# nintendops/DynamicFusion_Body

Hardware: AMD Instinct MI355X
Metric: Mvoxels/s TSDF fusion + GN-iters/s warp solve, 256³ grid, 1/2/4/8 GPU (higher is better)
Workload: dtype f64 geometry / f32 volume

## Files before the change

dynamicfusion_body_amd/csrc/dfh_common.h:

```cpp
#pragma once
#include <hip/hip_runtime.h>

#include <cstdarg>
#include <cstdio>

#include "../../include/dfusion_hip.h"

namespace dfh {

char *last_error_buf();
int fail(int code, const char *fmt, ...);

#define DFH_HIP_CHECK(expr)                                                               \
    do {                                                                                  \
        hipError_t _e = (expr);                                                           \
        if (_e != hipSuccess)                                                             \
            return ::dfh::fail(DFH_E_HIP, "%s failed: %s", #expr, hipGetErrorString(_e)); \
    } while (0)

#define DFH_REQUIRE(cond, ...)                                  \
    do {                                                        \
        if (!(cond)) return ::dfh::fail(DFH_E_BADARG, __VA_ARGS__); \
    } while (0)

inline int check_slab(const char *what, const dfh_slab *s) {
    DFH_REQUIRE(s, "%s: null slab", what);
    DFH_REQUIRE(s->res[0] > 0 && s->res[1] > 0 && s->res[2] > 0, "%s: bad grid %dx%dx%d", what, s->res[0], s->res[1], s->res[2]);
    DFH_REQUIRE(0 <= s->x0 && s->x0 <= s->x1 && s->x1 <= s->res[0], "%s: slab [%d,%d) outside [0,%d)", what, s->x0, s->x1, s->res[0]);
    DFH_REQUIRE(s->x1 - s->x0 <= 65535, "%s: slab has more than 65535 planes", what);
    return DFH_OK;
}

inline int check_volume(const char *what, const dfh_volume *v) {
    DFH_REQUIRE(v && v->tsdf && v->tsdf_w, "%s: null volume", what);
    DFH_REQUIRE(v->dtype == DFH_F32 || v->dtype == DFH_F64, "%s: bad volume dtype %d", what, v->dtype);
    return check_slab(what, &v->slab);
}

struct Mat3 { double m[9]; };
struct Mat34 { double m[12]; };
struct Vec3 { double v[3]; };
struct DQ { double q[8]; };

constexpr int kWave = 64;
#ifndef DFH_GN_TILE
#define DFH_GN_TILE 128
#endif
constexpr int kGnTile = DFH_GN_TILE;

#define DFH_OPTION_LIST(X)                                                                                                \
    X(k1_strided) X(k1_late_loads) X(k1_planes_per_block) X(k1_force_scalar) X(k1_bricks_min) X(k1_no_bricks)            \
    X(k1_bricks_nocull) X(k1_no_multi) X(k1_cull) X(k1_nzi) X(k1_prefetch) X(k1_nt) X(k1_gather_first)                  \
    X(k2_exact) X(k2_no_strided) X(k2_nt) X(k3_no_cache) X(k3_exact) X(k3_no_lds) X(k3_wg_per_cu) X(k3_tpb) X(k3_skip) X(plan_radix) X(rigid_atomic) X(gn_reg_own_launch) X(gn_reg_own_gather) \
    X(dbg_gather_part) X(pcg_wpb) X(pcg_multilaunch) X(pcg_spin_limit) X(pcg_one_xcd) X(gn_iter_own_clear) X(gn_gather_full) X(gn_no_view_cull)                                                            \
    X(py_plan_torch) X(py_allreduce_full) X(py_gn_atomic) X(py_gn_no_fused_assoc) X(py_gn_no_fused_iter) X(py_gn_iter_per_call) X(py_no_side_stream) X(py_no_host_scalars) \
    X(k12_store) X(nd_path) X(raycast_skip)
struct Options {
#define DFH_X(n) long n;
    DFH_OPTION_LIST(DFH_X)
#undef DFH_X
};
const Options &opt();

struct DeviceInfo {
    int n_cu = 0;
    int pcg_occ512 = -1, pcg_occ1024 = -1;
};
DeviceInfo &device_info(int device);
inline bool on(long v) { return v > 0; }

}
```

dynamicfusion_body_amd/csrc/dfh_fuse_volume.hip:

```cpp
#include "dfh_warped_views.h"

#include <algorithm>
#include <cmath>
#include <cstdlib>
#include <mutex>
#include <unordered_map>

namespace dfh {

template <typename T, int N>
struct alignas(sizeof(T) * N) VPack {
    T v[N];
};

struct RigidParams {
    DQ lw;
    double tdist, wmax;
    int X, Y, Z;
    int LX, LY, LZ;
    int x0, nx;
    int zpacks, zp_shift;
};

__device__ __forceinline__ void pack_coords2(int zpacks, int zp_shift, int &y, int &zp) {
    const int lin = blockIdx.x * 256 + threadIdx.x;
    if (zp_shift >= 0) {
        y = lin >> zp_shift;
        zp = lin & ((1 << zp_shift) - 1);
    } else {
        y = lin / zpacks;
        zp = lin - y * zpacks;
    }
}

template <typename VolT, typename LiveT, int VEC>
__global__ __launch_bounds__(256) void fuse_volume_rigid_kernel(VolT *__restrict__ tsdf, VolT *__restrict__ tsdf_w,
                                                                 const LiveT *__restrict__ live, const RigidParams p) {
    int y, zp;
    pack_coords2(p.zpacks, p.zp_shift, y, zp);
    if (y >= p.Y) return;
    const int xl = blockIdx.y;
    const int x = p.x0 + xl;
    const int z0 = zp * VEC;
    double sv[VEC];
    bool upd[VEC];
    bool any = false;
#pragma unroll
    for (int j = 0; j < VEC; ++j) {
        const int z = z0 + j;
        const D3 q = dqb_warp_exact(p.lw.q, (double)x, (double)y, (double)z);
        double s = 0.0;
        bool ok = (z < p.Z) && interpolate_exact(live, p.LX, p.LY, p.LZ, q.x, q.y, q.z, s);
        ok = ok && (s > -1.0 * p.tdist);
        sv[j] = s;
        upd[j] = ok;
        any = any | ok;
    }
    if (!any) return;
    const size_t off = ((size_t)xl * p.Y + y) * p.Z + z0;
    using P = VPack<VolT, VEC>;
    P t = *reinterpret_cast<const P *>(tsdf + off);
    P w = *reinterpret_cast<const P *>(tsdf_w + off);
#pragma unroll
    for (int j = 0; j < VEC; ++j) {
        if (upd[j]) {
            const double wt = (double)w.v[j];
            const double m = sv[j] < p.tdist ? sv[j] : p.tdist;
            t.v[j] = (VolT)(((double)t.v[j] * wt + m * 1.0) / (1.0 + wt));
            const double nw = 1.0 + wt;
            w.v[j] = (VolT)(nw < p.wmax ? nw : p.wmax);
        }
    }
    *reinterpret_cast<P *>(tsdf + off) = t;
    *reinterpret_cast<P *>(tsdf_w + off) = w;
}

struct RigidFastParams {
    double M[9], t[3];
};

template <typename LiveT>
__device__ __forceinline__ double sample_fast(const LiveT *__restrict__ vol, int RY, int RZ, double px, double py, double pz) {
    const double fx = floor(px), fy = floor(py), fz = floor(pz);
    const int x0 = (int)fx, y0 = (int)fy, z0 = (int)fz;
    const int x1 = (int)ceil(px), y1 = (int)ceil(py), z1 = (int)ceil(pz);
    const double xd = px - fx, yd = py - fy, zd = pz - fz;
    const size_t sx = (size_t)RY * RZ, sy = (size_t)RZ;
    const double c000 = (double)vol[x0 * sx + y0 * sy + z0], c100 = (double)vol[x1 * sx + y0 * sy + z0];
    const double c001 = (double)vol[x0 * sx + y1 * sy + z0], c101 = (double)vol[x1 * sx + y1 * sy + z0];
    const double c010 = (double)vol[x0 * sx + y0 * sy + z1], c110 = (double)vol[x1 * sx + y0 * sy + z1];
    const double c011 = (double)vol[x0 * sx + y1 * sy + z1], c111 = (double)vol[x1 * sx + y1 * sy + z1];
    const double c00 = __builtin_fma(xd, c100 - c000, c000), c01 = __builtin_fma(xd, c101 - c001, c001);
    const double c10 = __builtin_fma(xd, c110 - c010, c010), c11 = __builtin_fma(xd, c111 - c011, c011);
    const double c0 = __builtin_fma(yd, c10 - c00, c00);
    const double c1 = __builtin_fma(yd, c11 - c01, c01);
    return __builtin_fma(zd, c1 - c0, c0);
}

template <typename LiveT, bool STRIDED, bool NT = false>
__global__ __launch_bounds__(256) void fuse_volume_rigid_fast_kernel(float *__restrict__ tsdf, float *__restrict__ tsdf_w,
                                                                      const LiveT *__restrict__ live, const RigidParams p,
                                                                      const RigidFastParams f) {
    constexpr int VEC = 4;
    int y, zp;
    pack_coords2(p.zpacks, p.zp_shift, y, zp);
    if (y >= p.Y) return;
    const int xl = blockIdx.y;
    const int x = p.x0 + xl;
    const int lane = threadIdx.x & 63;
    const int z0 = STRIDED ? (zp - lane) * VEC + lane : zp * VEC;
    constexpr int ZS = STRIDED ? 64 : 1;
    const double xf = (double)x, yf = (double)y, zf = (double)z0;
    double q[3];
#pragma unroll
    for (int r = 0; r < 3; ++r)
        q[r] = __builtin_fma(f.M[3 * r + 2], zf, __builtin_fma(f.M[3 * r + 1], yf, __builtin_fma(f.M[3 * r], xf, f.t[r])));
    const double hx = (double)(p.LX - 1), hy = (double)(p.LY - 1), hz = (double)(p.LZ - 1);
    const float tdf = (float)p.tdist;
    float mv[VEC];
    bool upd[VEC];
    bool any = false;
#pragma unroll
    for (int j = 0; j < VEC; ++j) {
        const double jf = (double)(j * ZS);
        const double qx = __builtin_fma(f.M[2], jf, q[0]), qy = __builtin_fma(f.M[5], jf, q[1]), qz = __builtin_fma(f.M[8], jf, q[2]);
        const double lo = fmin(fmin(qx, qy), qz);
        const double hi = fmin(fmin(hx - qx, hy - qy), hz - qz);
        const double edge = fmin(fabs(lo), fabs(hi));
        bool ok = (lo >= 0.0) & (hi >= 0.0);
        bool redo = (int)!(fmin(fmin(fabs(qx), fabs(qy)), fabs(qz)) > 1e-9) | (int)!(fmin(fmin(fabs(hx - qx), fabs(hy - qy)), fabs(hz - qz)) > 1e-9);
        (void)edge;
        double sv = 0.0;
        if (ok) {
            const double fx = qx - floor(qx), fy = qy - floor(qy), fz = qz - floor(qz);
            redo = redo | !(fmin(fmin(fmin(fx, fy), fz), fmin(fmin(1.0 - fx, 1.0 - fy), 1.0 - fz)) > 1e-9);
            sv = sample_fast(live, p.LY, p.LZ, qx, qy, qz);
            const double margin = sv + p.tdist;
            ok = margin > 0.0;
            redo = redo | !(fabs(margin) > 1e-9 * (1.0 + fabs(sv)));
        }
        if (__builtin_expect(redo, 0)) {
            int xx = x, yy = y, zz = z0 + j * ZS;
            asm volatile("" : "+v"(xx), "+v"(yy), "+v"(zz));
            const D3 e = dqb_warp_exact(p.lw.q, (double)xx, (double)yy, (double)zz);
            ok = interpolate_exact(live, p.LX, p.LY, p.LZ, e.x, e.y, e.z, sv) && (sv > -1.0 * p.tdist);
        }
        ok = ok & (z0 + j * ZS < p.Z);
        mv[j] = (float)(sv < p.tdist ? sv : p.tdist);
        upd[j] = ok;
        any = any | ok;
    }
    (void)tdf;
    if (!any) return;
    const size_t off = ((size_t)xl * p.Y + y) * p.Z + z0;
    using P = VPack<float, VEC>;
    P t, w;
    if (STRIDED) {
#pragma unroll
        for (int j = 0; j < VEC; ++j) {
            if (NT) { t.v[j] = __builtin_nontemporal_load(tsdf + off + j * ZS); w.v[j] = __builtin_nontemporal_load(tsdf_w + off + j * ZS); }
            else { t.v[j] = tsdf[off + j * ZS]; w.v[j] = tsdf_w[off + j * ZS]; }
        }
    } else {
        t = *reinterpret_cast<const P *>(tsdf + off);
        w = *reinterpret_cast<const P *>(tsdf_w + off);
    }
    const float wmaxf = (float)p.wmax;
#pragma unroll
    for (int j = 0; j < VEC; ++j) {
        const float wt = w.v[j];
        const float d = wt + 1.0f;
        const float n = fmaf(t.v[j], wt, mv[j]);
        const float r = __builtin_amdgcn_rcpf(d);
        float qn = n * r;
        qn = fmaf(fmaf(-d, qn, n), r, qn);
        t.v[j] = upd[j] ? qn : t.v[j];
        w.v[j] = upd[j] ? fminf(d, wmaxf) : wt;
    }
    if (STRIDED) {
#pragma unroll
        for (int j = 0; j < VEC; ++j) {
            if (upd[j]) {
                if (NT) { __builtin_nontemporal_store(t.v[j], tsdf + off + j * ZS); __builtin_nontemporal_store(w.v[j], tsdf_w + off + j * ZS); }
                else { tsdf[off + j * ZS] = t.v[j]; tsdf_w[off + j * ZS] = w.v[j]; }
            }
        }
    } else {
        *reinterpret_cast<P *>(tsdf + off) = t;
        *reinterpret_cast<P *>(tsdf_w + off) = w;
    }
}

static void fold_rigid(const double *q, RigidFastParams &f) {
    const double w = q[0], x = q[1], y = q[2], z = q[3];
    f.M[0] = w * w + x * x - y * y - z * z; f.M[1] = 2 * (x * y - w * z);           f.M[2] = 2 * (x * z + w * y);
    f.M[3] = 2 * (x * y + w * z);           f.M[4] = w * w - x * x + y * y - z * z; f.M[5] = 2 * (y * z - w * x);
    f.M[6] = 2 * (x * z - w * y);           f.M[7] = 2 * (y * z + w * x);           f.M[8] = w * w - x * x - y * y + z * z;
    const double d0 = q[4], d1 = q[5], d2 = q[6], d3 = q[7];
    f.t[0] = 2 * (-d0 * x + d1 * w - d2 * z + d3 * y);
    f.t[1] = 2 * (-d0 * y + d1 * z + d2 * w - d3 * x);
    f.t[2] = 2 * (-d0 * z - d1 * y + d2 * x + d3 * w);
}

template <typename VolT, typename LiveT>
static int launch_rigid(void *tsdf, void *tsdf_w, const void *live, RigidParams &p, bool vec4, hipStream_t s) {
    p.zpacks = vec4 ? p.Z / 4 : p.Z;
    p.zp_shift = -1;
    for (int b = 0; b < 31; ++b) if (p.zpacks == (1 << b)) p.zp_shift = b;
    const long per_plane = (long)p.Y * p.zpacks;
    dim3 grid((unsigned)((per_plane + 255) / 256), (unsigned)p.nx), block(256);
    if (vec4) {
        hipLaunchKernelGGL((fuse_volume_rigid_kernel<VolT, LiveT, 4>), grid, block, 0, s, (VolT *)tsdf, (VolT *)tsdf_w,
                           (const LiveT *)live, p);
    } else {
        hipLaunchKernelGGL((fuse_volume_rigid_kernel<VolT, LiveT, 1>), grid, block, 0, s, (VolT *)tsdf, (VolT *)tsdf_w,
                           (const LiveT *)live, p);
    }
    DFH_HIP_CHECK(hipGetLastError());
    return DFH_OK;
}

#define DFH_BRICK_RADIUS 7.7942286340599480
#define DFH_SAMPLE_MARGIN 1.7320508075688774

__global__ __launch_bounds__(256) void dqb_candidates_kernel(const double *__restrict__ node_pos, int *__restrict__ cand,
                                                              const DqbParams p) {
    const long brick = (long)blockIdx.x * 256 + threadIdx.x;
    const long nbricks = (long)p.nbx * p.nby * p.nbz;
    if (brick >= nbricks) return;
    const int bz = (int)(brick % p.nbz);
    const int by = (int)((brick / p.nbz) % p.nby);
    const int bx = (int)(brick / ((long)p.nbz * p.nby));
    const double lx = (double)(p.x0 + bx * kBX), ly = (double)(by * kBY), lz = (double)(bz * kBZ);
    const double hx = lx + (kBX - 1), hy = ly + (kBY - 1), hz = lz + (kBZ - 1);
    const double cx = 0.5 * (lx + hx), cy = 0.5 * (ly + hy), cz = 0.5 * (lz + hz);
    double bd[kKMax];
    int bi[kKMax];
#pragma unroll
    for (int i = 0; i < kKMax; ++i) { bd[i] = __builtin_huge_val(); bi[i] = -1; }
    for (int n = 0; n < p.N; ++n) {
        const double dx = cx - node_pos[3 * n], dy = cy - node_pos[3 * n + 1], dz = cz - node_pos[3 * n + 2];
        const double d2 = (dx * dx + dy * dy) + dz * dz;
        if (d2 < bd[kKMax - 1]) topk_insert<kKMax>(bd, bi, d2, n);
    }
    const double R = sqrt(select_k<kKMax>(bd, p.k)) + DFH_BRICK_RADIUS + DFH_SAMPLE_MARGIN + 1e-6;
    const double R2 = R * R;
    int *c = cand + brick * (kCap + 1);
    int cnt = 0;
    for (int n = 0; n < p.N; ++n) {
        const double qx = node_pos[3 * n], qy = node_pos[3 * n + 1], qz = node_pos[3 * n + 2];
        const double dx = fmax(fmax(lx - qx, qx - hx), 0.0), dy = fmax(fmax(ly - qy, qy - hy), 0.0), dz = fmax(fmax(lz - qz, qz - hz), 0.0);
        const double d2 = (dx * dx + dy * dy) + dz * dz;
        if (d2 <= R2) {
            if (cnt < kCap) c[1 + cnt] = n;
            ++cnt;
        }
    }
    c[0] = cnt <= kCap ? cnt : -1;
}


template <typename VolT, typename LiveT, int KS, int MODE>
__global__ __launch_bounds__(256) void fuse_volume_dqb_kernel(VolT *__restrict__ tsdf, VolT *__restrict__ tsdf_w,
                                                               const LiveT *__restrict__ live,
                                                               const double *__restrict__ node_pos,
                                                               const double *__restrict__ node_dq,
                                                               const double *__restrict__ node_w,
                                                               const int *__restrict__ cand,
                                                               unsigned short *__restrict__ knn_cache,
                                                               double *__restrict__ w_cache, const DqbParams p) {
    const size_t nvox = (size_t)p.nx * p.Y * p.Z;
    const long brick = blockIdx.x;
    int xl, y, z;
    bool inb;
    if (MODE >= 2) {
        const size_t lin = (size_t)blockIdx.x * 256 + threadIdx.x;
        inb = lin < nvox;
        z = (int)(lin % (size_t)p.Z);
        y = (int)((lin / (size_t)p.Z) % (size_t)p.Y);
        xl = (int)(lin / ((size_t)p.Z * p.Y));
    } else {
        const int bz = (int)(brick % p.nbz);
        const int by = (int)((brick / p.nbz) % p.nby);
        const int bx = (int)(brick / ((long)p.nbz * p.nby));
        const int lz = threadIdx.x & (kBZ - 1);
        const int ly = (threadIdx.x >> 4) & (kBY - 1);
        const int lx = threadIdx.x >> 6;
        xl = bx * kBX + lx; y = by * kBY + ly; z = bz * kBZ + lz;
        inb = (xl < p.nx) && (y < p.Y) && (z < p.Z);
    }
    const double px = (double)(p.x0 + xl), py = (double)y, pz = (double)z;
    const size_t off = ((size_t)xl * p.Y + y) * p.Z + z;
    double bd[KS];
    int bi[KS];
    double wg[KS];
    double wi;
    if (MODE >= 2) {
        if (!inb) return;
        unsigned short id[KS];
        if (KS == 4 && p.k == 4) {
            const uint2 v = *reinterpret_cast<const uint2 *>(knn_cache + off * 4);
            id[0] = (unsigned short)(v.x & 0xffffu); id[1] = (unsigned short)(v.x >> 16);
            id[2] = (unsigned short)(v.y & 0xffffu); id[3] = (unsigned short)(v.y >> 16);
        } else {
#pragma unroll
            for (int j = 0; j < KS; ++j) id[j] = j < p.k ? knn_cache[off * p.k + j] : (unsigned short)0;
        }
#pragma unroll
        for (int j = 0; j < KS; ++j) bi[j] = min((int)id[j], p.N - 1);
        if (MODE == 3) {
#pragma unroll
            for (int j = 0; j < KS; ++j) wg[j] = j < p.k ? w_cache[(size_t)j * nvox + off] : 0.0;
            wi = w_cache[(size_t)p.k * nvox + off];
        } else {
#pragma unroll
            for (int j = 0; j < KS; ++j) {
                const int gi = bi[j];
                const double dx = px - node_pos[3 * gi], dy = py - node_pos[3 * gi + 1], dz = pz - node_pos[3 * gi + 2];
                bd[j] = (dx * dx + dy * dy) + dz * dz;
// ... 886 lines not shown
                                   p, sk, redo_list, (unsigned)(nv / 4), sat_ok);
            else
                hipLaunchKernelGGL(dqb_stream_kernel<false>, dim3((unsigned)((nv / 4 + 255) / 256)), dim3(256), 0, s, (float *)tsdf, (float *)tsdf_w, wi_cache,
                                   p, sk, redo_list, (unsigned)(nv / 4), sat_ok);
        }
#define DFH_K3L(TPB, STRIDE)                                                                                                                          \
        do {                                                                                                                                          \
            if (skip) hipLaunchKernelGGL((fuse_volume_dqb_lds_kernel<LiveT, TPB, STRIDE, true>), dim3((unsigned)wgs), dim3(TPB), lds, s, (float *)tsdf,  \
                                         (float *)tsdf_w, (const LiveT *)live, node_pos, node_dq, node_w, knn_cache, w_cache, p, f, (int)n_runs,        \
                                         redo_list, (const unsigned *)sk.sub_count, (const unsigned *)sk.sub_list, sk.sub_cap);                       \
            else hipLaunchKernelGGL((fuse_volume_dqb_lds_kernel<LiveT, TPB, STRIDE, false>), dim3((unsigned)wgs), dim3(TPB), lds, s, (float *)tsdf,     \
                                    (float *)tsdf_w, (const LiveT *)live, node_pos, node_dq, node_w, knn_cache, w_cache, p, f, (int)n_runs, redo_list, \
                                    (const unsigned *)nullptr, (const unsigned *)nullptr, 0u);                                                       \
        } while (0)
        if (big) DFH_K3L(1024, kDqLdsStrideBig);
        else if (tpb == 256) DFH_K3L(256, kDqLdsStride); else if (tpb == 512) DFH_K3L(512, kDqLdsStride); else DFH_K3L(1024, kDqLdsStride);
        hipLaunchKernelGGL((dqb_redo_kernel<LiveT>), dim3(kRedoBlocks), dim3(256), 0, s, (float *)tsdf, (float *)tsdf_w, (const LiveT *)live, node_pos, node_dq,
                           node_w, knn_cache, reinterpret_cast<const float *>(w_cache + 3 * ((size_t)p.nx * p.Y * p.Z)), p, redo_list);
#undef DFH_K3L
    } else if (mode == 0) DFH_K3F(0); else if (mode == 1) DFH_K3F(1); else if (mode == 2) DFH_K3F(2); else DFH_K3F(3);
#undef DFH_K3F
    if (mode == 1 && w_cache && skip_sizes_ok(p)) {
        DqbSkip sk = {};
        if (skip_layout(p, w_cache, sk))
            hipLaunchKernelGGL(dqb_used_nodes_kernel, dim3((unsigned)nbricks), dim3(256), 0, s, (const unsigned short *)knn_cache, (const int *)cand, p, sk);
    }
    DFH_HIP_CHECK(hipGetLastError());
    return DFH_OK;
}

template <typename VolT, typename LiveT>
static int launch_dqb(void *tsdf, void *tsdf_w, const void *live, const double *node_pos, const double *node_dq,
                      const double *node_w, int *cand, unsigned short *knn_cache, double *w_cache, int mode, const DqbParams &p,
                      hipStream_t s) {
    const long nbricks = (long)p.nbx * p.nby * p.nbz;
    const long nblocks = mode >= 2 ? ((long)p.nx * p.Y * p.Z + 255) / 256 : nbricks;
#define DFH_K3(KS, MODE) hipLaunchKernelGGL((fuse_volume_dqb_kernel<VolT, LiveT, KS, MODE>), dim3((unsigned)nblocks), dim3(256), 0, s, \
                                            (VolT *)tsdf, (VolT *)tsdf_w, (const LiveT *)live, node_pos, node_dq, node_w, cand, knn_cache, w_cache, p)
    if (p.k <= 4) {
        if (mode == 0) DFH_K3(4, 0); else if (mode == 1) DFH_K3(4, 1); else if (mode == 2) DFH_K3(4, 2); else DFH_K3(4, 3);
    } else {
        if (mode == 0) DFH_K3(kKMax, 0); else if (mode == 1) DFH_K3(kKMax, 1); else if (mode == 2) DFH_K3(kKMax, 2); else DFH_K3(kKMax, 3);
    }
#undef DFH_K3
    DFH_HIP_CHECK(hipGetLastError());
    return DFH_OK;
}


static std::mutex &dqb_format_mutex() { static std::mutex mu; return mu; }
static std::unordered_map<const void *, int> &dqb_format_map() { static std::unordered_map<const void *, int> format; return format; }

void dqb_forget_weights(const void *workspace) {
    std::lock_guard<std::mutex> lock(dqb_format_mutex());
    dqb_format_map().erase(workspace);
}

static int check_live(const char *what, const dfh_live *l) {
    DFH_REQUIRE(l && l->data, "%s: null live volume", what);
    DFH_REQUIRE(l->dtype == DFH_F32 || l->dtype == DFH_F64, "%s: bad live dtype %d", what, l->dtype);
    DFH_REQUIRE(l->res[0] > 0 && l->res[1] > 0 && l->res[2] > 0, "%s: bad live grid", what);
    return DFH_OK;
}

template <int KS>
__global__ __launch_bounds__(256) void sample_knn_bricks_kernel(const double *__restrict__ spos, int S,
                                                                 const double *__restrict__ node_pos,
                                                                 const double *__restrict__ node_w,
                                                                 const int *__restrict__ cand, const DqbParams p,
                                                                 int *__restrict__ nbr, double *__restrict__ wts) {
    const int i = blockIdx.x * 256 + threadIdx.x;
    if (i >= S) return;
    const double px = spos[3 * (size_t)i], py = spos[3 * (size_t)i + 1], pz = spos[3 * (size_t)i + 2];
    const double rx = rint(px), ry = rint(py), rz = rint(pz);
    const bool inside = rx >= (double)p.x0 && rx < (double)(p.x0 + p.nx) && ry >= 0.0 && ry < (double)p.Y && rz >= 0.0 &&
                        rz < (double)p.Z;
    const int *c = nullptr;
    int cnt = -1;
    if (inside) {
        const long brick = ((long)(((int)rx - p.x0) / kBX) * p.nby + (int)ry / kBY) * p.nbz + (int)rz / kBZ;
        c = cand + brick * (kCap + 1);
        cnt = c[0];
    }
    double bd[KS];
    int bi[KS];
#pragma unroll
    for (int j = 0; j < KS; ++j) { bd[j] = __builtin_huge_val(); bi[j] = -1; }
    const int total = cnt >= 0 ? cnt : p.N;
    constexpr int U = 8;
    for (int j0 = 0; j0 < total; j0 += U) {
        int g[U];
        double x[U], y[U], z[U];
#pragma unroll
        for (int u = 0; u < U; ++u) {
            const int jj = min(j0 + u, total - 1);
            g[u] = cnt >= 0 ? c[1 + jj] : jj;
        }
#pragma unroll
        for (int u = 0; u < U; ++u) { x[u] = node_pos[3 * g[u]]; y[u] = node_pos[3 * g[u] + 1]; z[u] = node_pos[3 * g[u] + 2]; }
#pragma unroll
        for (int u = 0; u < U; ++u) {
            const double dx = px - x[u], dy = py - y[u], dz = pz - z[u];
            const double d2 = (dx * dx + dy * dy) + dz * dz;
            if (j0 + u < total && d2 < bd[KS - 1]) topk_insert<KS>(bd, bi, d2, g[u]);
        }
    }
    bool full = true;
#pragma unroll
    for (int j = 0; j < KS; ++j) full = full && (j >= p.k || bi[j] >= 0);
    if (!full) {
        for (int j = 0; j < p.k; ++j) { nbr[(size_t)i * p.k + j] = j; wts[(size_t)i * p.k + j] = 0.0; }
        return;
    }
#pragma unroll
    for (int j = 0; j < KS; ++j) {
        if (j < p.k) {
            const int gi = bi[j];
            nbr[(size_t)i * p.k + j] = gi;
            const double t = sqrt(bd[j]) / (2.0 * node_w[gi]);
            wts[(size_t)i * p.k + j] = exp(-1.0 * (t * t));
        }
    }
}

}

extern "C" int dfh_fuse_volume_rigid(const dfh_volume *vol, const dfh_live *live_vol, const double lw_dq[8], double tdist, double wmax,
                                     void *stream) {
    using namespace dfh;
    int rc = check_volume("dfh_fuse_volume_rigid", vol);
    if (rc == DFH_OK) rc = check_live("dfh_fuse_volume_rigid", live_vol);
    if (rc != DFH_OK) return rc;
    DFH_REQUIRE(lw_dq, "dfh_fuse_volume_rigid: null pointer");
    DFH_REQUIRE((long)live_vol->res[0] * live_vol->res[1] * live_vol->res[2] < (1L << 40), "dfh_fuse_volume_rigid: live grid too large");
    if (vol->slab.x1 == vol->slab.x0) return DFH_OK;
    void *tsdf = vol->tsdf, *tsdf_w = vol->tsdf_w;
    const void *live = live_vol->data;
    const int vol_dtype = vol->dtype, live_dtype = live_vol->dtype;
    RigidParams p;
    for (int i = 0; i < 8; ++i) p.lw.q[i] = lw_dq[i];
    p.tdist = tdist; p.wmax = wmax;
    set_grid(p, vol->slab, live_vol->res);
    const size_t esz = vol_dtype == DFH_F32 ? 4 : 8;
    const bool vec4 = (p.Z % 4 == 0) && ((uintptr_t)tsdf % (4 * esz) == 0) && ((uintptr_t)tsdf_w % (4 * esz) == 0);
    hipStream_t s = static_cast<hipStream_t>(stream);
    if (vol_dtype == DFH_F32 && vec4 && !on(opt().k2_exact)) {
        RigidFastParams f;
        fold_rigid(lw_dq, f);
        p.zpacks = p.Z / 4;
        p.zp_shift = -1;
        for (int b = 0; b < 31; ++b) if (p.zpacks == (1 << b)) p.zp_shift = b;
        dim3 grid((unsigned)(((long)p.Y * p.zpacks + 255) / 256), (unsigned)p.nx), block(256);
        const bool strided = p.zpacks % 64 == 0 && !on(opt().k2_no_strided);
#define DFH_K2(LT, ST, NT_) hipLaunchKernelGGL((fuse_volume_rigid_fast_kernel<LT, ST, NT_>), grid, block, 0, s, (float *)tsdf, \
                                               (float *)tsdf_w, (const LT *)live, p, f)
        const bool nt = strided && (opt().k2_nt > 0 || (opt().k2_nt < 0 && (size_t)p.nx * p.Y * p.Z * 8 > ((size_t)256 << 20)));
        if (live_dtype == DFH_F32) { if (strided) { if (nt) DFH_K2(float, true, true); else DFH_K2(float, true, false); } else DFH_K2(float, false, false); }
        else { if (strided) { if (nt) DFH_K2(double, true, true); else DFH_K2(double, true, false); } else DFH_K2(double, false, false); }
#undef DFH_K2
        DFH_HIP_CHECK(hipGetLastError());
        return DFH_OK;
    }
    if (vol_dtype == DFH_F32) {
        if (live_dtype == DFH_F32) return launch_rigid<float, float>(tsdf, tsdf_w, live, p, vec4, s);
        return launch_rigid<float, double>(tsdf, tsdf_w, live, p, vec4, s);
    }
    if (live_dtype == DFH_F32) return launch_rigid<double, float>(tsdf, tsdf_w, live, p, vec4, s);
    return launch_rigid<double, double>(tsdf, tsdf_w, live, p, vec4, s);
}

extern "C" size_t dfh_dqb_workspace_bytes(const dfh_slab *slab) {
    if (dfh::check_slab("dfh_dqb_workspace_bytes", slab) != DFH_OK || slab->x1 == slab->x0) return 0;
    return dfh::cand_bytes(*slab);
}

extern "C" size_t dfh_dqb_workspace_bytes_cached(const dfh_slab *slab, int knn, int n_nodes, int level) {
    if (dfh::check_slab("dfh_dqb_workspace_bytes_cached", slab) != DFH_OK || slab->x1 == slab->x0) return 0;
    const size_t base = dfh::cand_bytes(*slab);
    if (level < 1 || knn < 1 || knn > dfh::kKMax || n_nodes > 65536) return base;
    const size_t nvox = (size_t)(slab->x1 - slab->x0) * slab->res[1] * slab->res[2];
    const size_t idx = (nvox * knn * sizeof(unsigned short) + 15) & ~(size_t)15;
    return base + idx + (level >= 2 ? nvox * (knn + 1) * sizeof(double) : 0);
}

extern "C" int dfh_fuse_volume_dqb(const dfh_volume *vol, const dfh_live *live_vol, const dfh_nodes *nodes, const double lw_dq[8],
                                   double tdist, double wmax, void *workspace, size_t workspace_bytes, int rebuild_candidates,
                                   void *stream) {
    using namespace dfh;
    int rc = check_volume("dfh_fuse_volume_dqb", vol);
    if (rc == DFH_OK) rc = check_live("dfh_fuse_volume_dqb", live_vol);
    if (rc != DFH_OK) return rc;
    DFH_REQUIRE(nodes && lw_dq && nodes->pos && nodes->dq && nodes->w, "dfh_fuse_volume_dqb: null pointer");
    const int knn = nodes->knn, n_nodes = nodes->n_nodes;
    DFH_REQUIRE(knn >= 1 && knn <= kKMax, "dfh_fuse_volume_dqb: knn=%d outside [1,%d]", knn, kKMax);
    DFH_REQUIRE(n_nodes >= knn, "dfh_fuse_volume_dqb: %d nodes < knn=%d", n_nodes, knn);
    const dfh_slab *sl = &vol->slab;
    if (sl->x1 == sl->x0) return DFH_OK;
    DFH_REQUIRE(workspace && workspace_bytes >= dfh_dqb_workspace_bytes(sl),
                "dfh_fuse_volume_dqb: workspace too small (need %zu bytes)", dfh_dqb_workspace_bytes(sl));
    void *tsdf = vol->tsdf, *tsdf_w = vol->tsdf_w;
    const void *live = live_vol->data;
    const double *node_pos = nodes->pos, *node_dq = nodes->dq, *node_w = nodes->w;
    const int vol_dtype = vol->dtype, live_dtype = live_vol->dtype;
    DqbParams p = dqb_params(*sl, live_vol->res, n_nodes, knn);
    for (int i = 0; i < 8; ++i) p.lw.q[i] = lw_dq[i];
    p.tdist = tdist; p.wmax = wmax;
    const long nbricks = (long)p.nbx * p.nby * p.nbz;
    DFH_REQUIRE(nbricks < (1L << 31), "dfh_fuse_volume_dqb: too many bricks");
    hipStream_t s = static_cast<hipStream_t>(stream);
    int *cand = static_cast<int *>(workspace);
    size_t cached1;
    unsigned short *knn_cache = dqb_index_region(sl, knn, n_nodes, workspace, workspace_bytes, &cached1);
    const bool has_idx = knn_cache != nullptr;
    const bool has_w = has_idx && workspace_bytes >= dfh_dqb_workspace_bytes_cached(sl, knn, n_nodes, 2);
    double *w_cache = has_w ? reinterpret_cast<double *>(static_cast<char *>(workspace) + cached1) : nullptr;
    int mode = !has_idx ? 0 : (rebuild_candidates ? 1 : (has_w ? 3 : 2));
    const bool fast = vol_dtype == DFH_F32 && knn == 4 && !on(opt().k3_exact);
    if (has_w) {
        std::mutex &mu = dqb_format_mutex();
        std::unordered_map<const void *, int> &format = dqb_format_map();
        std::lock_guard<std::mutex> lock(mu);
        if (mode == 1) {
            if (format.size() > 4096) format.clear();
            format[workspace] = fast ? 1 : 2;
        } else if (mode == 3) {
            const auto it = format.find(workspace);
            if (it == format.end() || it->second != (fast ? 1 : 2)) mode = 2;
        }
    }
    if (rebuild_candidates) {
        hipLaunchKernelGGL(dqb_candidates_kernel, dim3((unsigned)((nbricks + 255) / 256)), dim3(256), 0, s, node_pos, cand, p);
        DFH_HIP_CHECK(hipGetLastError());
    }
    if (fast) {
        if (live_dtype == DFH_F32) return launch_dqb_fast<float>(tsdf, tsdf_w, live, node_pos, node_dq, node_w, cand, knn_cache, w_cache, mode, p, s);
        return launch_dqb_fast<double>(tsdf, tsdf_w, live, node_pos, node_dq, node_w, cand, knn_cache, w_cache, mode, p, s);
    }
    if (vol_dtype == DFH_F32) {
        if (live_dtype == DFH_F32) return launch_dqb<float, float>(tsdf, tsdf_w, live, node_pos, node_dq, node_w, cand, knn_cache, w_cache, mode, p, s);
        return launch_dqb<float, double>(tsdf, tsdf_w, live, node_pos, node_dq, node_w, cand, knn_cache, w_cache, mode, p, s);
    }
    if (live_dtype == DFH_F32) return launch_dqb<double, float>(tsdf, tsdf_w, live, node_pos, node_dq, node_w, cand, knn_cache, w_cache, mode, p, s);
    return launch_dqb<double, double>(tsdf, tsdf_w, live, node_pos, node_dq, node_w, cand, knn_cache, w_cache, mode, p, s);
}

extern "C" int dfh_dqb_skip_layout(const dfh_slab *slab, const int live_res[3], int knn, int n_nodes, size_t out[13]) {
    using namespace dfh;
    const int rc = check_slab("dfh_dqb_skip_layout", slab);
    if (rc != DFH_OK) return rc;
    DFH_REQUIRE(live_res && out, "dfh_dqb_skip_layout: null pointer");
    DFH_REQUIRE(knn == 4, "dfh_dqb_skip_layout: the skip belongs to the knn = 4 float32 path");
    for (int i = 0; i < 13; ++i) out[i] = 0;
    if (slab->x1 == slab->x0) return DFH_OK;
    const DqbParams p = dqb_params(*slab, live_res, n_nodes, knn);
    const size_t cached1 = dfh_dqb_workspace_bytes_cached(slab, knn, n_nodes, 1);
    const size_t cached2 = dfh_dqb_workspace_bytes_cached(slab, knn, n_nodes, 2);
    DFH_REQUIRE(cached2 > cached1, "dfh_dqb_skip_layout: no level-2 workspace for these sizes");
    DqbSkip k = {};
    size_t used = 0;
    const bool fits = skip_layout(p, reinterpret_cast<double *>(cached1), k, &used);
    out[0] = reinterpret_cast<size_t>(k.U); out[1] = reinterpret_cast<size_t>(k.S); out[2] = reinterpret_cast<size_t>(k.mb);
    out[3] = reinterpret_cast<size_t>(k.db);
    out[6] = (size_t)k.CX; out[7] = (size_t)k.CY; out[8] = (size_t)k.WZ; out[9] = (size_t)k.SCX; out[10] = (size_t)k.SCY;
    out[11] = fits && skip_sizes_ok(p) ? 1 : 0;
    out[12] = reinterpret_cast<size_t>(k.used);
    return DFH_OK;
}

extern "C" int dfh_dqb_build_candidates(const dfh_slab *slab, const double *node_pos, int n_nodes, int knn,
                                        void *workspace, size_t workspace_bytes, void *stream) {
    using namespace dfh;
    const int rc = check_slab("dfh_dqb_build_candidates", slab);
    if (rc != DFH_OK) return rc;
    DFH_REQUIRE(node_pos, "dfh_dqb_build_candidates: null pointer");
    DFH_REQUIRE(knn >= 1 && knn <= kKMax && n_nodes >= knn, "dfh_dqb_build_candidates: knn=%d, %d nodes", knn, n_nodes);
    if (slab->x1 == slab->x0) return DFH_OK;
    DFH_REQUIRE(workspace && workspace_bytes >= dfh_dqb_workspace_bytes(slab),
                "dfh_dqb_build_candidates: workspace too small (need %zu bytes)", dfh_dqb_workspace_bytes(slab));
    const DqbParams p = dqb_params(*slab, nullptr, n_nodes, knn);
    const long nbricks = (long)p.nbx * p.nby * p.nbz;
    DFH_REQUIRE(nbricks < (1L << 31), "dfh_dqb_build_candidates: too many bricks");
    hipLaunchKernelGGL(dqb_candidates_kernel, dim3((unsigned)((nbricks + 255) / 256)), dim3(256), 0, static_cast<hipStream_t>(stream),
                       node_pos, static_cast<int *>(workspace), p);
    DFH_HIP_CHECK(hipGetLastError());
    return DFH_OK;
}

extern "C" int dfh_sample_knn_bricks(const double *sample_pos, int n_samples, const double *node_pos, const double *node_w,
                                     int n_nodes, int knn, const dfh_slab *slab, const void *workspace,
                                     size_t workspace_bytes, int *nbr_out, double *weights_out, void *stream) {
    using namespace dfh;
    const int rc = check_slab("dfh_sample_knn_bricks", slab);
    if (rc != DFH_OK) return rc;
    DFH_REQUIRE(n_samples >= 0, "dfh_sample_knn_bricks: negative sample count");
    if (n_samples == 0) return DFH_OK;
    DFH_REQUIRE(sample_pos && node_pos && node_w && nbr_out && weights_out, "dfh_sample_knn_bricks: null pointer");
    DFH_REQUIRE(knn >= 1 && knn <= kKMax && n_nodes >= knn, "dfh_sample_knn_bricks: knn=%d, %d nodes", knn, n_nodes);
    if (slab->x1 == slab->x0) return DFH_OK;
    DFH_REQUIRE(workspace && workspace_bytes >= dfh_dqb_workspace_bytes(slab),
                "dfh_sample_knn_bricks: workspace too small (need %zu bytes)", dfh_dqb_workspace_bytes(slab));
    const DqbParams p = dqb_params(*slab, nullptr, n_nodes, knn);
    dim3 grid((unsigned)((n_samples + 255) / 256)), block(256);
    hipStream_t s = static_cast<hipStream_t>(stream);
    if (knn <= 4)
        hipLaunchKernelGGL(sample_knn_bricks_kernel<4>, grid, block, 0, s, sample_pos, n_samples, node_pos, node_w,
                           static_cast<const int *>(workspace), p, nbr_out, weights_out);
    else
        hipLaunchKernelGGL(sample_knn_bricks_kernel<kKMax>, grid, block, 0, s, sample_pos, n_samples, node_pos, node_w,
                           static_cast<const int *>(workspace), p, nbr_out, weights_out);
// ... 4 lines not shown
```

Baseline: 510,500.

## Restructure rigid fusion kernel with integer guard checks and paired trilinear loads

Replaces the default rigid TSDF fusion kernel with a version that classifies each voxel by integer comparisons on the high words of its fractional coordinates and margin. Only near-boundary or ambiguous candidates fall back to an exact guarded recomputation. Trilinear corner loads are issued as z-adjacent pairs, batched across the four voxels, and separated by scheduling barriers so gathers overlap the TSDF reads. The old kernel stays available behind a legacy option. The aim is fewer double-precision comparisons and more memory-level parallelism, at the cost of extra registers and a rarely taken divergent slow path.

After: 510,300. About the same (-0.0%).

```diff
diff --git a/dynamicfusion_body_amd/csrc/dfh_common.h b/dynamicfusion_body_amd/csrc/dfh_common.h
--- a/dynamicfusion_body_amd/csrc/dfh_common.h
+++ b/dynamicfusion_body_amd/csrc/dfh_common.h
@@ -51,7 +51,7 @@
 #define DFH_OPTION_LIST(X)                                                                                                \
     X(k1_strided) X(k1_late_loads) X(k1_planes_per_block) X(k1_force_scalar) X(k1_bricks_min) X(k1_no_bricks)            \
     X(k1_bricks_nocull) X(k1_no_multi) X(k1_cull) X(k1_nzi) X(k1_prefetch) X(k1_nt) X(k1_gather_first)                  \
-    X(k2_exact) X(k2_no_strided) X(k2_nt) X(k3_no_cache) X(k3_exact) X(k3_no_lds) X(k3_wg_per_cu) X(k3_tpb) X(k3_skip) X(plan_radix) X(rigid_atomic) X(gn_reg_own_launch) X(gn_reg_own_gather) \
+    X(k2_exact) X(k2_no_strided) X(k2_nt) X(k2_legacy) X(k3_no_cache) X(k3_exact) X(k3_no_lds) X(k3_wg_per_cu) X(k3_tpb) X(k3_skip) X(plan_radix) X(rigid_atomic) X(gn_reg_own_launch) X(gn_reg_own_gather) \
     X(dbg_gather_part) X(pcg_wpb) X(pcg_multilaunch) X(pcg_spin_limit) X(pcg_one_xcd) X(gn_iter_own_clear) X(gn_gather_full) X(gn_no_view_cull)                                                            \
     X(py_plan_torch) X(py_allreduce_full) X(py_gn_atomic) X(py_gn_no_fused_assoc) X(py_gn_no_fused_iter) X(py_gn_iter_per_call) X(py_no_side_stream) X(py_no_host_scalars) \
     X(k12_store) X(nd_path) X(raycast_skip)
diff --git a/dynamicfusion_body_amd/csrc/dfh_fuse_volume.hip b/dynamicfusion_body_amd/csrc/dfh_fuse_volume.hip
--- a/dynamicfusion_body_amd/csrc/dfh_fuse_volume.hip
+++ b/dynamicfusion_body_amd/csrc/dfh_fuse_volume.hip
@@ -3,6 +3,7 @@
 #include <algorithm>
 #include <cmath>
 #include <cstdlib>
+#include <cstring>
 #include <mutex>
 #include <unordered_map>
 
@@ -98,7 +99,7 @@
 }
 
 template <typename LiveT, bool STRIDED, bool NT = false>
-__global__ __launch_bounds__(256) void fuse_volume_rigid_fast_kernel(float *__restrict__ tsdf, float *__restrict__ tsdf_w,
+__global__ __launch_bounds__(256) void fuse_volume_rigid_fast_legacy_kernel(float *__restrict__ tsdf, float *__restrict__ tsdf_w,
                                                                       const LiveT *__restrict__ live, const RigidParams p,
                                                                       const RigidFastParams f) {
     constexpr int VEC = 4;
@@ -165,6 +166,201 @@
         t = *reinterpret_cast<const P *>(tsdf + off);
         w = *reinterpret_cast<const P *>(tsdf_w + off);
     }
+    const float wmaxf = (float)p.wmax;
+#pragma unroll
+    for (int j = 0; j < VEC; ++j) {
+        const float wt = w.v[j];
+        const float d = wt + 1.0f;
+        const float n = fmaf(t.v[j], wt, mv[j]);
+        const float r = __builtin_amdgcn_rcpf(d);
+        float qn = n * r;
+        qn = fmaf(fmaf(-d, qn, n), r, qn);
+        t.v[j] = upd[j] ? qn : t.v[j];
+        w.v[j] = upd[j] ? fminf(d, wmaxf) : wt;
+    }
+    if (STRIDED) {
+#pragma unroll
+        for (int j = 0; j < VEC; ++j) {
+            if (upd[j]) {
+                if (NT) { __builtin_nontemporal_store(t.v[j], tsdf + off + j * ZS); __builtin_nontemporal_store(w.v[j], tsdf_w + off + j * ZS); }
+                else { tsdf[off + j * ZS] = t.v[j]; tsdf_w[off + j * ZS] = w.v[j]; }
+            }
+        }
+    } else {
+        *reinterpret_cast<P *>(tsdf + off) = t;
+        *reinterpret_cast<P *>(tsdf_w + off) = w;
+    }
+}
+
+struct RigidGuards {
+    unsigned long long gx, gy, gz;
+    unsigned c_lo, c_span;
+    unsigned d_lo, d_span;
+};
+
+static unsigned hi_word(double v) {
+    unsigned long long b;
+    std::memcpy(&b, &v, 8);
+    return (unsigned)(b >> 32);
+}
+
+static RigidGuards rigid_guards(double tdist, int LX, int LY, int LZ) {
+    RigidGuards g;
+    g.gx = LX > 1 ? (unsigned long long)LY * LZ : 0; g.gy = LY > 1 ? (unsigned long long)LZ : 0; g.gz = LZ > 1 ? 1 : 0;
+    g.c_lo = hi_word(1e-9) + 1u;
+    g.c_span = hi_word(0.999999998) - g.c_lo;
+    const double k = 2e-9 * (1.0 + std::fabs(tdist));
+    g.d_lo = hi_word(k) + 1u;
+    g.d_span = (k > 0.0 && k < 1e300) ? 0x7ff00000u - g.d_lo : 0u;
+    return g;
+}
+
+template <typename LiveT>
+__device__ __forceinline__ void rigid_voxel_guarded(const LiveT *__restrict__ live, const RigidParams &p, const RigidFastParams &f, int x, int y,
+                                                    int z0, int dz, bool &upd, float &mv) {
+    asm volatile("" : "+v"(x), "+v"(y), "+v"(z0));
+    const double xf = (double)x, yf = (double)y, zf = (double)z0, jf = (double)dz;
+    double q[3];
+#pragma unroll
+    for (int r = 0; r < 3; ++r)
+        q[r] = __builtin_fma(f.M[3 * r + 2], zf, __builtin_fma(f.M[3 * r + 1], yf, __builtin_fma(f.M[3 * r], xf, f.t[r])));
+    const double hx = (double)(p.LX - 1), hy = (double)(p.LY - 1), hz = (double)(p.LZ - 1);
+    const double qx = __builtin_fma(f.M[2], jf, q[0]), qy = __builtin_fma(f.M[5], jf, q[1]), qz = __builtin_fma(f.M[8], jf, q[2]);
+    const double lo = fmin(fmin(qx, qy), qz);
+    const double hi = fmin(fmin(hx - qx, hy - qy), hz - qz);
+    bool ok = (lo >= 0.0) & (hi >= 0.0);
+    bool redo = (int)!(fmin(fmin(fabs(qx), fabs(qy)), fabs(qz)) > 1e-9) | (int)!(fmin(fmin(fabs(hx - qx), fabs(hy - qy)), fabs(hz - qz)) > 1e-9);
+    double sv = 0.0;
+    if (ok) {
+        const double fx = qx - floor(qx), fy = qy - floor(qy), fz = qz - floor(qz);
+        redo = redo | !(fmin(fmin(fmin(fx, fy), fz), fmin(fmin(1.0 - fx, 1.0 - fy), 1.0 - fz)) > 1e-9);
+        sv = sample_fast(live, p.LY, p.LZ, qx, qy, qz);
+        const double margin = sv + p.tdist;
+        ok = margin > 0.0;
+        redo = redo | !(fabs(margin) > 1e-9 * (1.0 + fabs(sv)));
+    }
+    if (redo) {
+        const D3 e = dqb_warp_exact(p.lw.q, (double)x, (double)y, (double)(z0 + dz));
+        ok = interpolate_exact(live, p.LX, p.LY, p.LZ, e.x, e.y, e.z, sv) && (sv > -1.0 * p.tdist);
+    }
+    ok = ok & (z0 + dz < p.Z);
+    mv = (float)(sv < p.tdist ? sv : p.tdist);
+    upd = ok;
+}
+
+#ifndef DFH_K2_DEPTH
+#define DFH_K2_DEPTH 4
+#endif
+
+template <typename LiveT> struct CellPair;
+template <> struct CellPair<float> { typedef float type __attribute__((ext_vector_type(2), aligned(4))); };
+template <> struct CellPair<double> { typedef double type __attribute__((ext_vector_type(2), aligned(8))); };
+
+template <typename LiveT, bool STRIDED, bool NT, bool PAIR>
+__global__ __launch_bounds__(256) void fuse_volume_rigid_fast_kernel(float *__restrict__ tsdf, float *__restrict__ tsdf_w,
+                                                                      const LiveT *__restrict__ live, const RigidParams p,
+                                                                      const RigidFastParams f, const RigidGuards g) {
+    constexpr int VEC = 4;
+    int y, zp;
+    pack_coords2(p.zpacks, p.zp_shift, y, zp);
+    if (y >= p.Y) return;
+    const int xl = blockIdx.y;
+    const int x = p.x0 + xl;
+    const int lane = threadIdx.x & 63;
+    const int z0 = STRIDED ? (zp - lane) * VEC + lane : zp * VEC;
+    constexpr int ZS = STRIDED ? 64 : 1;
+    const double xf = (double)x, yf = (double)y, zf = (double)z0;
+    double q[3];
+#pragma unroll
+    for (int r = 0; r < 3; ++r)
+        q[r] = __builtin_fma(f.M[3 * r + 2], zf, __builtin_fma(f.M[3 * r + 1], yf, __builtin_fma(f.M[3 * r], xf, f.t[r])));
+    const unsigned hxi = (unsigned)(p.LX - 1), hyi = (unsigned)(p.LY - 1), hzi = (unsigned)(p.LZ - 1);
+    const size_t sx = (size_t)p.LY * p.LZ, sy = (size_t)p.LZ;
+    double xd[VEC], yd[VEC], zd[VEC];
+    bool hot[VEC], cand[VEC];
+    size_t e000[VEC];
+    bool work = false;
+#pragma unroll
+    for (int j = 0; j < VEC; ++j) {
+        const double jf = (double)(j * ZS);
+        const double qx = __builtin_fma(f.M[2], jf, q[0]), qy = __builtin_fma(f.M[5], jf, q[1]), qz = __builtin_fma(f.M[8], jf, q[2]);
+        const double fx = floor(qx), fy = floor(qy), fz = floor(qz);
+        xd[j] = qx - fx; yd[j] = qy - fy; zd[j] = qz - fz;
+        const int ix = (int)fx, iy = (int)fy, iz = (int)fz;
+        const unsigned wx = (unsigned)__double2hiint(xd[j]), wy = (unsigned)__double2hiint(yd[j]), wz = (unsigned)__double2hiint(zd[j]);
+        cand[j] = !((min(min(wx, wy), wz) - g.c_lo < g.c_span) & (max(max(wx, wy), wz) - g.c_lo < g.c_span));
+        hot[j] = !cand[j] && (unsigned)ix < hxi && (unsigned)iy < hyi && (unsigned)iz < hzi;
+        work = work | hot[j] | cand[j];
+        const int mx = hot[j] ? ix : 0, my = hot[j] ? iy : 0, mz = hot[j] ? iz : 0;
+        e000[j] = mx * sx + my * sy + mz;
+    }
+    if (!work) return;
+    const size_t off = ((size_t)xl * p.Y + y) * p.Z + z0;
+    using P = VPack<float, VEC>;
+    P t, w;
+    float mv[VEC];
+    bool upd[VEC];
+    bool any_cand = false;
+    constexpr int G = DFH_K2_DEPTH == 2 ? 2 : VEC;
+#pragma unroll
+    for (int g0 = 0; g0 < VEC; g0 += G) {
+        LiveT c[G][8];
+#pragma unroll
+        for (int i = 0; i < G; ++i) {
+            const int j = g0 + i;
+            const LiveT *b0 = live + e000[j];
+            if (PAIR) {
+                using C2 = typename CellPair<LiveT>::type;
+                const C2 v0 = *reinterpret_cast<const C2 *>(b0), v1 = *reinterpret_cast<const C2 *>(b0 + g.gx);
+                const C2 v2 = *reinterpret_cast<const C2 *>(b0 + g.gy), v3 = *reinterpret_cast<const C2 *>(b0 + (g.gy + g.gx));
+                c[i][0] = v0.x; c[i][1] = v1.x; c[i][2] = v2.x; c[i][3] = v3.x;
+                c[i][4] = v0.y; c[i][5] = v1.y; c[i][6] = v2.y; c[i][7] = v3.y;
+            } else {
+                const LiveT *b1 = b0 + g.gz;
+                c[i][0] = b0[0]; c[i][1] = b0[g.gx];
+                c[i][2] = b0[g.gy]; c[i][3] = b0[g.gy + g.gx];
+                c[i][4] = b1[0]; c[i][5] = b1[g.gx];
+                c[i][6] = b1[g.gy]; c[i][7] = b1[g.gy + g.gx];
+            }
+        }
+        if (g0 + G == VEC) {
+            if (STRIDED) {
+#pragma unroll
+                for (int j = 0; j < VEC; ++j) {
+                    if (NT) { t.v[j] = __builtin_nontemporal_load(tsdf + off + j * ZS); w.v[j] = __builtin_nontemporal_load(tsdf_w + off + j * ZS); }
+                    else { t.v[j] = tsdf[off + j * ZS]; w.v[j] = tsdf_w[off + j * ZS]; }
+                }
+            } else {
+                t = *reinterpret_cast<const P *>(tsdf + off);
+                w = *reinterpret_cast<const P *>(tsdf_w + off);
+            }
+        }
+        if (DFH_K2_DEPTH) __builtin_amdgcn_sched_barrier(0);
+#pragma unroll
+        for (int i = 0; i < G; ++i) {
+            const int j = g0 + i;
+            const double c000 = (double)c[i][0], c100 = (double)c[i][1], c001 = (double)c[i][2], c101 = (double)c[i][3];
+            const double c010 = (double)c[i][4], c110 = (double)c[i][5], c011 = (double)c[i][6], c111 = (double)c[i][7];
+            const double c00 = __builtin_fma(xd[j], c100 - c000, c000), c01 = __builtin_fma(xd[j], c101 - c001, c001);
+            const double c10 = __builtin_fma(xd[j], c110 - c010, c010), c11 = __builtin_fma(xd[j], c111 - c011, c011);
+            const double c0 = __builtin_fma(yd[j], c10 - c00, c00);
+            const double c1 = __builtin_fma(yd[j], c11 - c01, c01);
+            const double sv = __builtin_fma(zd[j], c1 - c0, c0);
+            const double margin = sv + p.tdist;
+            const unsigned wm = (unsigned)__double2hiint(margin) & 0x7fffffffu;
+            cand[j] = cand[j] | (hot[j] && wm - g.d_lo >= g.d_span);
+            upd[j] = hot[j] & (margin > 0.0);
+            mv[j] = (float)(sv < p.tdist ? sv : p.tdist);
+            any_cand = any_cand | cand[j];
+        }
+        if (DFH_K2_DEPTH == 2) __builtin_amdgcn_sched_barrier(0);
+    }
+    if (__builtin_expect(any_cand, 0)) {
+#pragma unroll
+        for (int j = 0; j < VEC; ++j)
+            if (cand[j]) rigid_voxel_guarded(live, p, f, x, y, z0, j * ZS, upd[j], mv[j]);
+    }
+    if (!(upd[0] | upd[1] | upd[2] | upd[3])) return;
     const float wmaxf = (float)p.wmax;
 #pragma unroll
     for (int j = 0; j < VEC; ++j) {
@@ -1357,9 +1553,22 @@
         for (int b = 0; b < 31; ++b) if (p.zpacks == (1 << b)) p.zp_shift = b;
         dim3 grid((unsigned)(((long)p.Y * p.zpacks + 255) / 256), (unsigned)p.nx), block(256);
         const bool strided = p.zpacks % 64 == 0 && !on(opt().k2_no_strided);
-#define DFH_K2(LT, ST, NT_) hipLaunchKernelGGL((fuse_volume_rigid_fast_kernel<LT, ST, NT_>), grid, block, 0, s, (float *)tsdf, \
+const bool nt = strided && (opt().k2_nt > 0 || (opt().k2_nt < 0 && (size_t)p.nx * p.Y * p.Z * 8 > ((size_t)256 << 20)));
+        if (on(opt().k2_legacy)) {
+#define DFH_K2(LT, ST, NT_) hipLaunchKernelGGL((fuse_volume_rigid_fast_legacy_kernel<LT, ST, NT_>), grid, block, 0, s, (float *)tsdf, \
                                                (float *)tsdf_w, (const LT *)live, p, f)
-        const bool nt = strided && (opt().k2_nt > 0 || (opt().k2_nt < 0 && (size_t)p.nx * p.Y * p.Z * 8 > ((size_t)256 << 20)));
+            if (live_dtype == DFH_F32) { if (strided) { if (nt) DFH_K2(float, true, true); else DFH_K2(float, true, false); } else DFH_K2(float, false, false); }
+            else { if (strided) { if (nt) DFH_K2(double, true, true); else DFH_K2(double, true, false); } else DFH_K2(double, false, false); }
+#undef DFH_K2
+            DFH_HIP_CHECK(hipGetLastError());
+            return DFH_OK;
+        }
+        const RigidGuards g = rigid_guards(tdist, p.LX, p.LY, p.LZ);
+        const bool pair = p.LZ > 1;
+#define DFH_K2(LT, ST, NT_) do { if (pair) hipLaunchKernelGGL((fuse_volume_rigid_fast_kernel<LT, ST, NT_, true>), grid, block, 0, s, (float *)tsdf, \
+                                                              (float *)tsdf_w, (const LT *)live, p, f, g);                                             \
+                                 else hipLaunchKernelGGL((fuse_volume_rigid_fast_kernel<LT, ST, NT_, false>), grid, block, 0, s, (float *)tsdf,        \
+                                                         (float *)tsdf_w, (const LT *)live, p, f, g); } while (0)
         if (live_dtype == DFH_F32) { if (strided) { if (nt) DFH_K2(float, true, true); else DFH_K2(float, true, false); } else DFH_K2(float, false, false); }
         else { if (strided) { if (nt) DFH_K2(double, true, true); else DFH_K2(double, true, false); } else DFH_K2(double, false, false); }
 #undef DFH_K2
```
